# aconley/mbb_emcee

Measured on AMD Instinct MI355X. Metric: walker-likelihood evals/sec (+ MCMC steps/sec), 250 walkers × 8 bands, 1/2/4/8 GPU, higher is better.
Workload: dtype f64; 1 GPU; cfg2/cfg3: 8 passbands (NQ 2209) with full response integration, thick+alpha, 250 walkers per GPU, device-resident stretch move; 1 step = 2 dependent half-steps; walkers_per_gpu=250, walkers=250, bands=8, nq=2209, sampler_form=form 7: one launch per <=4096 steps, preconditioning=50 ms of scratch-ensemble steps before the W warm-up steps (GPU clocks)

## Files before the change

mbb_emcee_amd/csrc/mbb_flowm.hip.h:

```cpp
#pragma once
#include "mbb_kernels.hip.h"

__device__ __forceinline__ long long flow_spin_limit(int spec_cfg)
{
    const int v = (spec_cfg >> 24) & 0x3f;
    return v == 63 ? 0ll : 1ll << (v ? v : 22);
}

constexpr int kFmReady = 0;
constexpr int kFmQDone = 4;
constexpr int kFmEDone = 8;
constexpr int kFmPen = 16;
constexpr int kFmStaged = 12;

__device__ __forceinline__ int fm_loop_lane(int l)
{
    asm volatile("" : "+v"(l));
    return l;
}
__device__ __forceinline__ void fm_put(double *pair, double v, unsigned long long tag)
{
    typedef unsigned int u32x4 __attribute__((ext_vector_type(4)));
    const unsigned long long vb = (unsigned long long)__double_as_longlong(v), chk = tag ^ vb;
    const u32x4 d = {(unsigned int)vb, (unsigned int)(vb >> 32), (unsigned int)chk, (unsigned int)(chk >> 32)};
    asm volatile("global_store_dwordx4 %0, %1, off sc1" : : "v"(pair), "v"(d) : "memory");
}
__device__ __forceinline__ bool fm_get(const double *pair, unsigned long long tag, double &v)
{
    typedef unsigned int u32x4 __attribute__((ext_vector_type(4)));
    u32x4 d;
    asm volatile("global_load_dwordx4 %0, %1, off sc1\n\ts_waitcnt vmcnt(0)" : "=v"(d) : "v"(pair) : "memory");
    const unsigned long long vb = ((unsigned long long)d.y << 32) | d.x, chk = ((unsigned long long)d.w << 32) | d.z;
    v = __longlong_as_double((long long)vb);
    return (chk ^ vb) == tag;
}

#define MBB_FM_COMMON() \
    const int nun = a.nunit, npart = a.npart, nb = a.nb; \
    const int wbase = ((int)blockIdx.x >> 1) * NP, cand = (int)blockIdx.x & 1; \
    WalkerK *wk0 = reinterpret_cast<WalkerK *>(smem_raw); \
    double *partial0 = reinterpret_cast<double *>(wk0 + NP * kFmNB); \
    double *mflux_all = partial0 + NP * kFmNB * (size_t)npart; \
    double *prop0 = mflux_all + 2 * nb; \
    double *s_flux = prop0 + NP * kFmNB * kFmProp; \
    double *s_ivar = s_flux + nb; \
    double *s_invcov = s_ivar + nb; \
    int2 *s_band = reinterpret_cast<int2 *>(s_invcov + (a.cov_in_lds ? (size_t)nb * nb : 0)); \
    double *cscr = reinterpret_cast<double *>(s_band + nb + 1); \
    int *ctl0 = reinterpret_cast<int *>(cscr + kFmNC * 64); \
    const size_t tab_off = ((size_t)(reinterpret_cast<unsigned char *>(ctl0 + 32 * NP) - smem_raw) + 15) & ~(size_t)15; \
    double *s_nu = reinterpret_cast<double *>(smem_raw + tab_off); \
    double *s_lnnu = s_nu + (STAGE ? a.nchunk * 64 : 0); \
    double *s_wt = s_lnnu + (STAGE ? a.nchunk * 64 : 0); \
    const long long spin_limit = flow_spin_limit(a.spec_cfg); \
    const FlowMView fv = flowm_view(a.spec, a.nw); \
    const unsigned long long serial32 = a.flow_serial << 32; \
    unsigned long long *const done_set = fv.done + (size_t)(a.spec_cfg & 1) * kFmRing * 16; \
    const int niter = a.persist;
#define MBB_FM_PAIRS_LOOP _Pragma("clang loop unroll(disable)")
#define MBB_FM_PAIR(vp) \
    const int w = wbase + (vp); \
    if constexpr (NP > 1) { if (w >= a.n) continue; }       \
    WalkerK *const wk = wk0 + (vp) * kFmNB; \
    double *const partial = partial0 + (size_t)(vp) * kFmNB * npart; \
    double *const prop = prop0 + (vp) * kFmNB * kFmProp; \
    int *const ctl = ctl0 + 32 * (vp); \
    (void)wk; (void)partial; (void)prop; (void)ctl
#define MBB_FM_ORDER() do { __builtin_amdgcn_fence(__ATOMIC_ACQ_REL, "wavefront"); __builtin_amdgcn_wave_barrier(); } while (0)
#define MBB_FM_WAITS() \
    auto dec_ok = [&](unsigned long long v, unsigned long long need) {    \
        return (v >> 32) == (serial32 >> 32) && ((v & 0xffffffffull) >> 1) >= need; \
    }; \
    auto lds_wait = [&](int *word, int need) { \
        long long spins = 0; \
        while (__hip_atomic_load(word, __ATOMIC_RELAXED, __HIP_MEMORY_SCOPE_WORKGROUP) < need) { \
            ++spins; \
            if (spins > spin_limit * 16 || \
                ((spins & 255) == 8 && __hip_atomic_load(a.errflag, __ATOMIC_RELAXED, __HIP_MEMORY_SCOPE_AGENT) != 0)) { \
                atomicMax(a.errflag, 9); \
                break; \
            } \
            __builtin_amdgcn_s_sleep(1); \
        } \
        MBB_FM_ORDER(); \
    }; \
    auto lds_post = [&](int *word, int v) { \
        MBB_FM_ORDER(); \
        __hip_atomic_store(word, v, __ATOMIC_RELAXED, __HIP_MEMORY_SCOPE_WORKGROUP); \
    }; \
    (void)dec_ok; (void)lds_wait; (void)lds_post
#ifdef MBB_WAVE_VECTOR
#define MBB_WAVE_ID(t) ((t) >> 6)
#else
#define MBB_WAVE_ID(t) __builtin_amdgcn_readfirstlane((t) >> 6)
#endif

template <bool OPTHIN, bool NOALPHA, bool STAGE, int NP>
__global__ void __launch_bounds__(1024) k_flowm(const LikeArgs a)
{
    static_assert(NP == 1, "one pair of walkers per workgroup (the two-pair shape is not built or tested any more)");
    CLikeArgs *const ka = MBB_KERNARGS();
    extern __shared__ __align__(16) unsigned char smem_raw[];
    __shared__ __align__(16) double s_tab[kExp2N];
    __shared__ __align__(16) double s_pb[kPolyBDoubles];
    __shared__ __align__(16) double s_pc[OPTHIN ? 2 : kPolyCDoubles];
    const int tid = threadIdx.x, lane = tid & 63, wave = MBB_WAVE_ID(tid);
    const int nwave = blockDim.x >> 6, nq = nwave - kFmNC - 2;
    const bool spread = nwave == 16;
    const int role = spread ? ((wave & 3) == 3 ? 1 + (wave >> 2) : (wave == 14 ? 2 + kFmNC : 0))
                            : (wave < nq ? 0 : 1 + wave - nq);
    const int qi = spread ? wave - (wave >> 2) : wave;
    {
        MBB_ROLE_ARGS();
        MBB_FM_COMMON();
        if (tid < 32 * NP) ctl0[tid] = 0;
        if (cand == 0 && tid < 12 * NP && wbase + tid / 12 < a.n) {
            const int t12 = tid % 12;
            const int r = (t12 < 6 ? 0 : a.c_count) + wbase + tid / 12, e = t12 < 6 ? t12 : t12 - 6;
            fm_put(fv.row + (size_t)r * kFmWords + 2 * e, a.pos6[(size_t)r * 6 + e], serial32);
        }
        if (blockIdx.x == 0 && tid < kFmRing * 16)
            __hip_atomic_store(fv.done + (size_t)((a.spec_cfg & 1) ^ 1) * kFmRing * 16 + tid, 0ull, __ATOMIC_RELAXED, __HIP_MEMORY_SCOPE_AGENT);
        (void)done_set; (void)niter; (void)spin_limit;
    }
    __syncthreads();
#ifdef MBB_STAMPS
    if (tid == 0 && a.stamps) a.stamps[(1u << 20) + 4096 + blockIdx.x] = __builtin_amdgcn_s_memrealtime();
    unsigned long long t_acc[8] = {0, 0, 0, 0, 0, 0, 0, 0};
    unsigned long long t_last = __builtin_amdgcn_s_memtime();
#define FM_T(kk) do { const unsigned long long t_now = __builtin_amdgcn_s_memtime(); t_acc[kk] += t_now - t_last; t_last = t_now; } while (0)
#define FM_TD(kk, dep) do { asm volatile("" ::"v"(dep)); FM_T(kk); } while (0)
#define FM_TOUT() do { if (lane == 0 && a.stamps) for (int kk = 0; kk < 8; ++kk) a.stamps[((size_t)blockIdx.x * 16 + wave) * 8 + kk] = t_acc[kk]; } while (0)
    if (lane == 0 && a.stamps) {
        unsigned hwid, xcc;
        asm volatile("s_getreg_b32 %0, hwreg(HW_REG_HW_ID)" : "=s"(hwid));
        asm volatile("s_getreg_b32 %0, hwreg(HW_REG_XCC_ID)" : "=s"(xcc));
        a.stamps[(1u << 20) + blockIdx.x * 16 + wave] = ((unsigned long long)xcc << 32) | hwid;
    }
#define FM_EV(jj, ev) do { if (lane == 0 && a.stamps && (jj) >= niter - 64) \
        a.stamps[(1u << 20) + 8192 + (((size_t)blockIdx.x * 64 + ((jj) & 63)) * 16 + (ev))] = __builtin_amdgcn_s_memrealtime(); } while (0)
#define FM_EVV(jj, ev, val) do { if (lane == 0 && a.stamps && (jj) >= niter - 64) \
        a.stamps[(1u << 20) + 8192 + (((size_t)blockIdx.x * 64 + ((jj) & 63)) * 16 + (ev))] = (unsigned long long)(val); } while (0)
#else
#define FM_EV(jj, ev) do { } while (0)
#define FM_EVV(jj, ev, val) do { } while (0)
#define FM_T(kk) do { } while (0)
#define FM_TD(kk, dep) do { } while (0)
#define FM_TOUT() do { } while (0)
#endif

    if (role == 0 || role > kFmNC) {
        MBB_ROLE_ARGS();
        MBB_FM_COMMON();
        MBB_FM_WAITS();
        const int ns = nq + 2, si = role == 0 ? qi : nq + (role - 1 - kFmNC);
        const int t0 = si * 64 + lane, nt = ns * 64;
        const double2 *gb = reinterpret_cast<const double2 *>(a.poly_b);
        const double2 *gc = reinterpret_cast<const double2 *>(a.poly_c);
        double2 *lb = reinterpret_cast<double2 *>(s_pb);
        double2 *lc = reinterpret_cast<double2 *>(s_pc);
        for (int i = t0; i < kExp2N; i += nt) s_tab[i] = kExp2Tab[i];
        for (int i = t0; i < kPolyBDoubles / 2; i += nt) lb[i] = gb[i];
        if (!OPTHIN)
            for (int i = t0; i < kPolyCDoubles / 2; i += nt) lc[i] = gc[i];
        for (int bb = t0; bb < nb; bb += nt) { s_flux[bb] = a.flux[bb]; s_ivar[bb] = a.ivar[bb]; s_band[bb] = a.band_rng[bb]; }
        if (a.cov_in_lds)
            for (int i = t0; i < nb * nb; i += nt) s_invcov[i] = a.invcov[i];
        if (STAGE) {
            const int n2 = a.nchunk * 32;
            const double2 *g0 = reinterpret_cast<const double2 *>(a.nu), *g1 = reinterpret_cast<const double2 *>(a.lnnu),
                          *g2 = reinterpret_cast<const double2 *>(a.wt);
            double2 *l0 = reinterpret_cast<double2 *>(s_nu), *l1 = reinterpret_cast<double2 *>(s_lnnu),
                    *l2 = reinterpret_cast<double2 *>(s_wt);
            for (int i = t0; i < n2; i += nt) { l0[i] = g0[i]; l1[i] = g1[i]; l2[i] = g2[i]; }
        }
        asm volatile("s_waitcnt vmcnt(0) lgkmcnt(0)" ::: "memory");
        MBB_FM_ORDER();
        if (lane == 0) __hip_atomic_fetch_add(ctl0 + kFmStaged, 1, __ATOMIC_RELAXED, __HIP_MEMORY_SCOPE_WORKGROUP);
        lds_wait(ctl0 + kFmStaged, ns);
    }
    if (role != 0) __builtin_amdgcn_s_setprio(3);
    if (role == 0) {
        MBB_ROLE_ARGS();
        MBB_FM_COMMON();
        MBB_FM_WAITS();
        MBB_PIN(a.unit_tab); MBB_PIN(a.tail_slot); MBB_PIN(a.errflag);
        if (!STAGE) { MBB_PIN(a.nu); MBB_PIN(a.lnnu); MBB_PIN(a.wt); }
        auto T_nu = [&](int i) { if constexpr (STAGE) return s_nu[i]; else return a.nu[i]; };
        auto T_ln = [&](int i) { if constexpr (STAGE) return s_lnnu[i]; else return a.lnnu[i]; };
        auto T_wt = [&](int i) { if constexpr (STAGE) return s_wt[i]; else return a.wt[i]; };
        const SampleTabs tabs = {s_tab, s_pb, s_pc};
        int4 us_first = make_int4(0, 0, 0, 0);
        if (qi < nun) us_first = a.unit_tab[qi];
        int tail_first = -1;
        if (qi < nun && us_first.w == 2) tail_first = a.tail_slot[4 * us_first.x + (lane >> 4)];
        for (int it = 0; it < niter; ++it)
        MBB_FM_PAIRS_LOOP
        for (int vp = 0; vp < NP; ++vp) {
            MBB_FM_PAIR(vp);
            const int b = it & (kFmNB - 1);
            lds_wait(ctl + kFmReady + b, it + 1);
            FM_T(0);
            if (qi == 1) FM_EV(it, 14);
            const WalkerK *wkb = wk + b;
            double *part = partial + (size_t)b * npart;
            if (wkb->status == ROW_OK) {
                const WalkerK k = *wkb;
                for (int u = qi; u < nun; u += nq) {
                    const int4 us = (u == qi) ? us_first : a.unit_tab[u];
                    const int s = us.x, c0 = us.y, c1 = us.z;
                    double acc = 0.0;
                    int c = c0;
                    for (; c + 2 <= c1; c += 2) {
                        const int i0 = c * 64 + lane, i1 = i0 + 64;
                        const double n0 = T_nu(i0), l0 = T_ln(i0), q0 = T_wt(i0);
                        const double n1 = T_nu(i1), l1 = T_ln(i1), q1 = T_wt(i1);
                        const double f0 = fnu_sample<OPTHIN, NOALPHA, true, false>(k, n0, l0, &tabs);
                        const double f1 = fnu_sample<OPTHIN, NOALPHA, true, false>(k, n1, l1, &tabs);
                        acc = fma(f0, q0, acc);
                        acc = fma(f1, q1, acc);
                    }
                    if (c < c1) {
                        const int i = c * 64 + lane;
                        const double f = fnu_sample<OPTHIN, NOALPHA, true, false>(k, T_nu(i), T_ln(i), &tabs);
                        acc = fma(f, T_wt(i), acc);
                    }
                    if (us.w == 0) {
                        acc = wave_sum_l63(acc);
                        if (lane == 63) part[s] = acc;
                    } else if (us.w == 2) {
                        acc = row_sum(acc);
                        if ((lane & 15) == 0) {
                            const int sl = (u == qi) ? tail_first : a.tail_slot[4 * s + (lane >> 4)];
                            if (sl >= 0) part[sl] = acc;
                        }
                    } else {
                        part[s + lane] = acc;
                    }
                }
            }
            MBB_FM_ORDER();
#ifdef MBB_STAMPS
            if (lane == 0) {
                const int cnt = __hip_atomic_fetch_add(ctl + kFmQDone + b, 1, __ATOMIC_RELAXED, __HIP_MEMORY_SCOPE_WORKGROUP);
                if (cnt + 1 == nq * ((it / kFmNB) + 1)) FM_EV(it, 15);
            }
#else
            if (lane == 0) __hip_atomic_fetch_add(ctl + kFmQDone + b, 1, __ATOMIC_RELAXED, __HIP_MEMORY_SCOPE_WORKGROUP);
#endif
            FM_T(1);
        }
        FM_TOUT();
        return;
    }

    if (role > kFmNC) {
        MBB_ROLE_ARGS();
        MBB_FM_COMMON();
        MBB_FM_WAITS();
        MBB_PIN(a.n); MBB_PIN(a.nw); MBB_PIN(a.c_count); MBB_PIN(a.step); MBB_PIN(a.seed); MBB_PIN(a.stretch_a);
        MBB_PIN(a.has_gprior); MBB_PIN(a.invcov); MBB_PIN(a.cov_in_lds); MBB_PIN(a.pos6); MBB_PIN(a.chain6);
        MBB_PIN(a.nacc); MBB_PIN(a.errflag);
        double *mflux = mflux_all + (size_t)(role - 1 - kFmNC) * nb;
        for (int it = role - 1 - kFmNC; it < niter; it += 2)
        MBB_FM_PAIRS_LOOP
        for (int vp = 0; vp < NP; ++vp) {
            MBB_FM_PAIR(vp);
            const int b = it & (kFmNB - 1);
            const int L_step = a.step + (it >> 1), L_half = it & 1;
            const unsigned long long L_seed = a.seed + 0x9E3779B97F4A7C15ull * (unsigned long long)(it >> 1);
            const int row = (L_half ? a.c_count : 0) + w, c_begin = L_half ? 0 : a.c_count;
            double zz, u3;
            int pj;
            stretch_draw(row, L_step, L_half, L_seed, a.stretch_a, a.c_count, zz, pj, u3);
            const int prow = c_begin + pj;
            const int m_par = flow_cnt(L_half ^ 1, it), m_s = flow_cnt(L_half, it);
            const unsigned long long need_p = (unsigned long long)flow_seq(L_half ^ 1, m_par);
            const double *lnp_p = fv.row + ((size_t)(m_s % kFmSlots) * a.nw + row) * kFmWords + 10;
            const unsigned long long tag_s = serial32 | (unsigned long long)flow_seq(L_half, m_s);
            const unsigned long long need_g = 2ull * (unsigned long long)a.n * (unsigned long long)(((it - kFmLag) / kFmRing) + 1);
            const unsigned long long *word = lane == 22 ? fv.mseq + (size_t)prow * kFmMseq + (m_par % kFmSlots)
                                                        : done_set + ((it - kFmLag) & (kFmRing - 1)) * 16;
            const bool watch = (lane == 22 && need_p > 0) || (lane == 23 && it >= kFmLag);
            const WalkerK *wkb = wk + b;
            const double *pr = prop + b * kFmProp;
            int st = ROW_SKIP;
            double cbb = 0.0, pen_u = 0.0, pen_g = 0.0, lnz4 = 0.0, lnu = 0.0, acc = 0.0;
            double q[5] = {0.0, 0.0, 0.0, 0.0, 0.0}, old5[5] = {0.0, 0.0, 0.0, 0.0, 0.0};
            auto sums = [&]() {
                lds_wait(ctl + kFmPen + b, it + 1);
                st = wkb->status;
                cbb = wkb->cq; pen_u = pr[7]; pen_g = pr[8];
#pragma unroll
                for (int i = 0; i < 5; ++i) { q[i] = pr[i]; old5[i] = pr[9 + i]; }
                lnz4 = pr[5]; lnu = pr[6];
                if (st == ROW_OK) {
                    const double *pj2 = partial + (size_t)b * npart;
                    auto band = [&](const int bb) {
                        double sum = 0.0;
                        const int2 rng = s_band[bb];
                        for (int sg = rng.x; sg < rng.y; sg += 4) {
                            const int l = rng.y - 1;
                            const double q0 = pj2[sg], q1 = pj2[min(sg + 1, l)], q2 = pj2[min(sg + 2, l)], q3 = pj2[min(sg + 3, l)];
                            sum += q0;
                            if (sg + 1 < rng.y) sum += q1;
                            if (sg + 2 < rng.y) sum += q2;
                            if (sg + 3 < rng.y) sum += q3;
                        }
                        sum *= cbb;
                        const double d = s_flux[bb] - sum;
                        if (a.invcov) mflux[bb] = d;
                        else acc = fma(d * d, s_ivar[bb], acc);
                    };
                    for (int bb = lane; bb < nb; bb += 64) band(bb);
                    if (a.invcov) {
                        MBB_FM_ORDER();
                        for (int i = lane; i < nb; i += 64) {
                            double t = 0.0;
                            const double *crow = (a.cov_in_lds ? s_invcov : a.invcov) + (size_t)i * nb;
                            for (int jj = 0; jj < nb; ++jj) t = fma(crow[jj], mflux[jj], t);
                            acc = fma(mflux[i], t, acc);
                        }
                    }
                    acc = (nb <= 16) ? wave_sum_row0(acc) : wave_sum(acc);
                }
                MBB_FM_ORDER();
                if (lane == 0) lds_post(ctl + kFmEDone + b, it + 1);
            };
            const int q_need = nq * ((it / kFmNB) + 1);
            FM_EV(it, 9);
#ifdef MBB_STAMPS
            unsigned long long t_ok = 0;
#endif
            unsigned long long pv = 0;
            double lnp = 0.0;
            bool ok = !(watch || lane == 21), have_sums = false;
            long long spins = 0;
            for (;;) {
                double lv = 0.0;
                unsigned long long lchk = 0, wv = 0;
                const bool ask_l = lane == 21 && !ok, ask_w = watch && !ok;
                if (ask_l) {
                    lv = ld_dev(lnp_p);
                    lchk = __hip_atomic_load(reinterpret_cast<const unsigned long long *>(lnp_p) + 1, __ATOMIC_RELAXED, __HIP_MEMORY_SCOPE_AGENT);
                }
                if (ask_w) wv = __hip_atomic_load(word, __ATOMIC_RELAXED, __HIP_MEMORY_SCOPE_AGENT);
                if (!have_sums && __hip_atomic_load(ctl + kFmQDone + b, __ATOMIC_RELAXED, __HIP_MEMORY_SCOPE_WORKGROUP) >= q_need) {
                    MBB_FM_ORDER();
                    FM_EV(it, 4);
                    sums();
                    have_sums = true;
                }
                if (ask_l) { lnp = lv; ok = (lchk ^ (unsigned long long)__double_as_longlong(lv)) == tag_s; }
                if (ask_w) { pv = wv; ok = lane == 22 ? dec_ok(pv, need_p) : pv >= need_g; }
#ifdef MBB_STAMPS
                if ((ask_l || ask_w) && ok) t_ok = __builtin_amdgcn_s_memrealtime();
#endif
                if (__builtin_amdgcn_ballot_w64(!ok) == 0) break;
                ++spins;
                if (spins > spin_limit ||
                    ((spins & 255) == 8 && __hip_atomic_load(a.errflag, __ATOMIC_RELAXED, __HIP_MEMORY_SCOPE_AGENT) != 0)) {
                    atomicMax(a.errflag, 9);
                    break;
                }
                __builtin_amdgcn_s_sleep(1);
            }
            const int flag = (need_p > 0 && (__shfl(pv, 22) & 1ull)) ? 1 : 0;
            const bool mine = flag == cand;
            const double lnp_cur = __shfl(lnp, 21);
            FM_TD(0, lnp_cur);
            FM_EV(it, 5);
            FM_EVV(it, 7, prow);
#ifdef MBB_STAMPS
            { const unsigned long long t21 = __shfl(t_ok, 21), t22 = __shfl(t_ok, 22), t23 = __shfl(t_ok, 23);
              FM_EVV(it, 10, t21); FM_EVV(it, 11, t22); FM_EVV(it, 12, t23); }
#endif
            if (!have_sums) {
                lds_wait(ctl + kFmQDone + b, q_need);
                FM_T(1);
                FM_EV(it, 4);
                sums();
            }
            FM_TD(2, acc);
            {
                double r;
                if (st == ROW_BELOW_LOWLIM) r = -__builtin_inf();
                else if (st != ROW_OK) r = __builtin_nan("");
                else {
                    r = fma(-0.5, acc, pen_u);
                    if (a.has_gprior) r += pen_g;
                }
                if (mine) {
                    if (lane == 0 && (st >= 2 || r != r)) atomicMax(a.errflag, (st >= 2 && st <= (int)ROW_NONFINITE) ? st : (int)ROW_NONFINITE);
                    const bool accept = (lnz4 + r - lnp_cur) > lnu;
                    const int m_new = m_s + 1;
                    FM_EV(it, 6);
                    if (lane == 0)
                        __hip_atomic_store(fv.mseq + (size_t)row * kFmMseq + (m_new % kFmSlots),
                                           serial32 | (2ull * (unsigned long long)(it + 1) + (accept ? 1ull : 0ull)), __ATOMIC_RELAXED,
                                           __HIP_MEMORY_SCOPE_AGENT);
                    const double lnp_new = accept ? r : lnp_cur;
                    double ve = lnp_new;
#pragma unroll
                    for (int i = 0; i < 5; ++i) ve = ((lane & 7) == i) ? (accept ? q[i] : old5[i]) : ve;
                    if (lane < 6) {
                        fm_put(fv.row + ((size_t)(m_new % kFmSlots) * a.nw + row) * kFmWords + 2 * lane, ve,
                               serial32 | (unsigned long long)(it + 1));
                        if (it + 2 >= niter) a.pos6[(size_t)row * 6 + lane] = ve;
                    }
                    else if (lane >= 8 && lane < 14 && a.chain6)
                        a.chain6[((size_t)it * a.n + w) * 6 + (lane - 8)] = ve;
                    if (lane == 0 && accept) atomicAdd(a.nacc + (size_t)L_half * a.n + w, 1u);
                }
                if (lane == 0) __hip_atomic_fetch_add(done_set + (it & (kFmRing - 1)) * 16, 1ull, __ATOMIC_RELAXED, __HIP_MEMORY_SCOPE_AGENT);
            }
            FM_T(3);
        }
        FM_TOUT();
        return;
    }

    {
        MBB_ROLE_ARGS();
        MBB_FM_COMMON();
        MBB_FM_WAITS();
        MBB_PIN(a.c_count); MBB_PIN(a.step); MBB_PIN(a.seed); MBB_PIN(a.stretch_a); MBB_PIN(a.nw); MBB_PIN(a.errflag); MBB_PIN(a.zpow);
        MBB_PIN(a.lowlim[0]); MBB_PIN(a.lowlim[1]); MBB_PIN(a.lowlim[2]); MBB_PIN(a.lowlim[3]); MBB_PIN(a.lowlim[4]);
        MBB_PIN(a.nunorm); MBB_PIN(a.lnunorm); MBB_PIN(a.has_uplim); MBB_PIN(a.has_gprior);
        const int cb = role - 1;
        const int lane_w = lane;
        double *scr = cscr + (size_t)cb * 64;
        auto spin = [&](const unsigned long long *word, unsigned long long need, bool watch) {
            unsigned long long v = 0;
            long long spins = 0;
            for (;;) {
                bool ok = true;
                if (watch) { v = __hip_atomic_load(word, __ATOMIC_RELAXED, __HIP_MEMORY_SCOPE_AGENT); ok = dec_ok(v, need); }
                if (__builtin_amdgcn_ballot_w64(!ok) == 0) break;
                ++spins;
                if (spins > spin_limit ||
                    ((spins & 255) == 8 && __hip_atomic_load(a.errflag, __ATOMIC_RELAXED, __HIP_MEMORY_SCOPE_AGENT) != 0)) {
                    atomicMax(a.errflag, 9);
                    break;
                }
                __builtin_amdgcn_s_sleep(1);
            }
            return v;
        };
        for (int j = cb; j < niter; j += kFmNC)
        MBB_FM_PAIRS_LOOP
        for (int vp = 0; vp < NP; ++vp) {
            MBB_FM_PAIR(vp);
            const int lane = fm_loop_lane(lane_w);
            const int vrow = lane >> 4, l16 = lane & 15, base = lane & 48;
            const int hj = j & 1;
            const int sb = hj ? a.c_count : 0, ob = hj ? 0 : a.c_count;
            const int tn = a.step + (j >> 1);
            const unsigned long long seed_n = a.seed + 0x9E3779B97F4A7C15ull * (unsigned long long)(j >> 1);
            const int tp = a.step + ((j - 1) >> 1), hp = hj ^ 1;
            const unsigned long long seed_p = a.seed + 0x9E3779B97F4A7C15ull * (unsigned long long)((j - 1) >> 1);
            const bool c1 = cand && j > 0;
            const int rown = sb + w;
            double zz = 1.0, u3 = 0.5, zp = 1.0, up;
            int pj = 0, pjp = 0;
            stretch_draw(rown, tn, hj, seed_n, a.stretch_a, a.c_count, zz, pj, u3);
            if (c1) stretch_draw(ob + pj, tp, hp, seed_p, a.stretch_a, a.c_count, zp, pjp, up);
            const int m_s = flow_cnt(hj, j - 1), m_o = flow_cnt(hj ^ 1, j - 1);
            const int m_next = m_s + 1;
            const int g = j - 2;
            const int m_q = flow_cnt(hj ^ 1, g);
            const int pprow = sb + pjp, prow = ob + pj;
            int qr = 0, qp = 0;
            if (m_s > 0) {
                const int tg = a.step + (g >> 1);
                const unsigned long long seed_g = a.seed + 0x9E3779B97F4A7C15ull * (unsigned long long)(g >> 1);
                double u0, z0;
                stretch_draw(rown, tg, hj, seed_g, a.stretch_a, a.c_count, z0, qr, u0);
                if (c1) stretch_draw(pprow, tg, hj, seed_g, a.stretch_a, a.c_count, z0, qp, u0);
            }
            int snv_off = 0, cpv_off = 15;
            {
                const bool has = m_s > 0;
                const int so = (has ? m_s - 1 : 0) % kFmSlots;
                const unsigned long long tag_old = serial32 | (unsigned long long)flow_seq(hj, has ? m_s - 1 : 0);
                const unsigned long long tag_g = serial32 | (unsigned long long)(g + 1);
                const unsigned long long tag_o = serial32 | (unsigned long long)flow_seq(hj ^ 1, m_o);
                const double *src = fv.row;
                unsigned long long tag = 0, need = 0;
                const unsigned long long *wsrc = fv.mseq;
                int slot = -1, kind = 0;
                if (lane < 2) {
                    const int r = lane == 0 ? qr : qp;
                    wsrc = fv.mseq + (size_t)(ob + r) * kFmMseq + (m_q % kFmSlots);
                    need = (unsigned long long)flow_seq(hj ^ 1, m_q);
                    kind = (has && m_q > 0 && (lane == 0 || c1)) ? 1 : 0;
                } else if (lane < 7) {
                    src = fv.row + ((size_t)so * a.nw + rown) * kFmWords + 2 * (lane - 2); tag = tag_old; slot = lane - 2; kind = 2;
                } else if (lane < 12) {
                    src = fv.row + ((size_t)so * a.nw + pprow) * kFmWords + 2 * (lane - 7); tag = tag_old; slot = 15 + lane - 7; kind = c1 ? 2 : 0;
                } else if (lane < 17) {
                    src = fv.row + ((size_t)(m_o % kFmSlots) * a.nw + prow) * kFmWords + 2 * (lane - 12); tag = tag_o; slot = 30 + lane - 12; kind = 2;
                } else if (lane < 27) {
                    const int c = (lane - 17) / 5, i = (lane - 17) - 5 * c;
                    src = fv.prop + (((size_t)rown * kFmSlots + (m_s % kFmSlots)) * 2 + c) * kFmWords + 2 * i; tag = tag_g; slot = 5 + lane - 17;
                    kind = has ? 2 : 0;
                } else if (lane < 37) {
                    const int c = (lane - 27) / 5, i = (lane - 27) - 5 * c;
                    src = fv.prop + (((size_t)pprow * kFmSlots + (m_s % kFmSlots)) * 2 + c) * kFmWords + 2 * i; tag = tag_g; slot = 20 + lane - 27;
                    kind = (has && c1) ? 2 : 0;
                }
                FM_EV(j, 13);
                bool ok = kind == 0;
                double v = 0.0;
                unsigned long long dv = 0;
                long long spins = 0;
                for (;;) {
                    if (kind == 2 && !ok) ok = fm_get(src, tag, v);
                    if (kind == 1 && !ok) { dv = __hip_atomic_load(wsrc, __ATOMIC_RELAXED, __HIP_MEMORY_SCOPE_AGENT); ok = dec_ok(dv, need); }
                    if (__builtin_amdgcn_ballot_w64(!ok) == 0) break;
                    ++spins;
                    if (spins > spin_limit ||
                        ((spins & 255) == 8 && __hip_atomic_load(a.errflag, __ATOMIC_RELAXED, __HIP_MEMORY_SCOPE_AGENT) != 0)) {
                        atomicMax(a.errflag, 9);
                        break;
                    }
                    __builtin_amdgcn_s_sleep(1);
                }
                if (slot >= 0) scr[slot] = v;
                FM_TD(0, v);
                FM_EV(j, 0);
                FM_EVV(j, 8, (unsigned long long)prow | ((unsigned long long)pprow << 10) | ((unsigned long long)(ob + qr) << 20) |
                                 ((unsigned long long)(ob + qp) << 30) | ((unsigned long long)(c1 ? 1 : 0) << 40) | ((unsigned long long)(m_s > 0 ? 1 : 0) << 41));
                MBB_FM_ORDER();
                const int cr = (int)(__shfl(dv, 0) & 1ull), cp = (int)(__shfl(dv, 1) & 1ull);
                const bool ar_v = has && (vrow & 1), ap_v = has && c1 && (vrow & 2);
                snv_off = ar_v ? 5 + 5 * cr : 0;
                cpv_off = ap_v ? 20 + 5 * cp : 15;
            }
            double snv[5], cpos[5], cpv[5];
#pragma unroll
            for (int i = 0; i < 5; ++i) { snv[i] = scr[snv_off + i]; cpv[i] = scr[cpv_off + i]; cpos[i] = scr[30 + i]; }
            FM_T(1);
            if (c1) {
#pragma unroll
                for (int i = 0; i < 5; ++i) cpos[i] = stretch_q(cpv[i], cpos[i], zp);
            }
            double p[5];
#pragma unroll
            for (int i = 0; i < 5; ++i) p[i] = stretch_q(cpos[i], snv[i], zz);
            double lo[4];
            vlog<true>(lo, p[0], p[2], zz, u3);
            WalkerK k;
            k.hokt9 = k.lhokt9 = k.beta = k.bp3 = k.cq = k.alpha = k.lx0 = k.xmerge = k.cbb = k.cpl = k.kap = k.peak = 0.0;
            k.status = ROW_SKIP;
            k.pad = 0;
            double pen_u = 0.0, pen_g = 0.0;
            const double lT = lo[0], lL = lo[1];
            const unsigned long long *w2 = fv.mseq + (size_t)(l16 == 0 ? rown : pprow) * kFmMseq + (m_s % kFmSlots);
            const bool watch2 = m_s > 0 && (l16 == 0 || (l16 == 1 && c1));
            const unsigned long long need2 = (unsigned long long)flow_seq(hj, m_s);
            unsigned long long v2 = 0;
#define MBB_WC_AFTER_PROLOGUE if (watch2) v2 = __hip_atomic_load(w2, __ATOMIC_RELAXED, __HIP_MEMORY_SCOPE_AGENT);
#define MBB_WC_PENALTIES_LATER
#include "mbb_walker_consts.inc"
#undef MBB_WC_PENALTIES_LATER
#undef MBB_WC_AFTER_PROLOGUE
#ifdef MBB_STAMPS
            {
                asm volatile("" ::"v"(pen_u + pen_g + k.cbb));
                const unsigned long long dt = __builtin_amdgcn_s_memtime() - t_last;
                if (dt > t_acc[6]) t_acc[6] = dt;
                if (t_acc[7] == 0 || dt < t_acc[7]) t_acc[7] = dt;
            }
#endif
            FM_TD(2, pen_u + pen_g + k.cbb);
            FM_EV(j, 1);
            if (__builtin_amdgcn_ballot_w64(watch2 && !dec_ok(v2, need2)) != 0) v2 = spin(w2, need2, watch2);
            const bool ar = m_s > 0 && (__shfl(v2, base + 0) & 1ull), ap = m_s > 0 && c1 && (__shfl(v2, base + 1) & 1ull);
            const int vsel = (ar ? 1 : 0) | (ap ? 2 : 0);
            FM_TD(3, v2);
            FM_EV(j, 2);
            const int bj = j & (kFmNB - 1);
            if (j >= kFmNB) lds_wait(ctl + kFmEDone + bj, j - kFmNB + 1);
            FM_T(4);
            if (vrow == vsel && l16 == 0) {
                wk[bj] = k;
                double *pr = prop + bj * kFmProp;
#pragma unroll
                for (int i = 0; i < 5; ++i) { pr[i] = p[i]; pr[9 + i] = snv[i]; }
                pr[5] = a.zpow * lo[2];
                pr[6] = lo[3];
                lds_post(ctl + kFmReady + bj, j + 1);
#ifdef MBB_STAMPS
                if (a.stamps && j >= niter - 64)
                    a.stamps[(1u << 20) + 8192 + (((size_t)blockIdx.x * 64 + (j & 63)) * 16 + 3)] = __builtin_amdgcn_s_memrealtime();
#endif
                double *rec = fv.prop + (((size_t)rown * kFmSlots + (m_next % kFmSlots)) * 2 + cand) * kFmWords;
                const unsigned long long tag = serial32 | (unsigned long long)(j + 1);
#pragma unroll
                for (int i = 0; i < 5; ++i) fm_put(rec + 2 * i, p[i], tag);
            }
#include "mbb_walker_penalties.inc"
            if (vrow == vsel && l16 == 0) {
                double *pr = prop + bj * kFmProp;
                pr[7] = pen_u;
                pr[8] = pen_g;
                lds_post(ctl + kFmPen + bj, j + 1);
            }
            FM_T(5);
        }
        FM_TOUT();
    }
#undef FM_EV
#undef FM_EVV
#undef FM_T
#undef FM_TD
#undef FM_TOUT
}
```

mbb_emcee_amd/csrc/mbb_hip.hip:

```cpp
#include <hip/hip_runtime.h>
#include <dlfcn.h>
#include <math.h>
#include <stdint.h>
#include <stdio.h>
#include <stdlib.h>
#include <string.h>
#include <time.h>

#include <algorithm>
#include <functional>
#include <string>
#include <type_traits>
#include <atomic>
#include <chrono>
#include <mutex>
#include <thread>
#include <vector>

#include "../../include/mbb_hip.h"
#include "mbb_device.hip.h"
#include "mbb_kernels.hip.h"
#include "mbb_summary.hip.h"

#define MBB_FLOW_EXT(OT, NA)                                                    \
// ... 1188 lines not shown
        if ((rc = mbb_lnlike_batch(c, pos, R, lnp.data(), st.data(), nullptr))) return rc;
        for (int i = 0; i < R; ++i)
            if (st[i] >= 2) return fail(MBB_ERR_ARG, "initial position is not a valid SED or lnprob is NaN");
    }
    int nfree = 0;
    for (int src = 0; src < s->nsrc; ++src) {
        unsigned int mask = 0;
        const double *p0 = pos + (size_t)src * s->nw * 5;
        for (int w = 1; w < s->nw; ++w)
            for (int k = 0; k < 5; ++k)
                if (p0[(size_t)w * 5 + k] != p0[k]) mask |= 1u << k;
        const int nf = __builtin_popcount(mask);
        if (src > 0 && nf != nfree) return fail(MBB_ERR_ARG, "the sources' initial ensembles differ in the number of constant (fixed) columns");
        nfree = nf;
    }
    std::vector<double> rows((size_t)R * 6);
    for (int i = 0; i < R; ++i) {
        for (int k = 0; k < 5; ++k) rows[(size_t)i * 6 + k] = pos[(size_t)i * 5 + k];
        rows[(size_t)i * 6 + 5] = lnp[i];
        if (lnp[i] != lnp[i]) return fail(MBB_ERR_ARG, "initial lnprob is NaN");
    }
    HIPCHK(hipMemcpyAsync(s->d_pos6, rows.data(), rows.size() * sizeof(double),
                          hipMemcpyHostToDevice, c->stream));
    HIPCHK(hipStreamSynchronize(c->stream));
    if (s->lost || s->unchecked) {
        HIPCHK(hipMemset(s->d_err, 0, sizeof(int)));
        s->lost = s->unchecked = false;
        s->spec_form = 0;
    }
    s->zpow = nfree > 1 ? (double)(nfree - 1) : 0.0;
    return MBB_OK;
}

static int sampler_check_pending(mbb_ctx *c, mbb_sampler_state *s)
{
    if (s->unchecked) {
        int err = 0;
        HIPCHK(hipMemcpyAsync(&err, s->d_err, sizeof(int), hipMemcpyDeviceToHost, c->stream));
        HIPCHK(hipStreamSynchronize(c->stream));
        s->unchecked = false;
        if (err == 9) {
            HIPCHK(hipMemset(s->d_err, 0, sizeof(int)));
            s->lost = true;
            s->spec_form = 0;
        }
    }
    if (s->lost)
        return fail(MBB_ERR_STATE, "the one-launch sampler run timed out waiting for a half-step; the ensemble it "
                                   "left behind is not a state of the chain: set the sampler's state again");
    return MBB_OK;
}

struct ShardPlan { int shards, first, last, per; bool collective, xchg; };

static int shard_plan(const mbb_ctx *c, const mbb_sampler_state *s, ShardPlan &p)
{
    const int half = s->nw / 2;
    const bool xchg = c->x.connected && !s->pos6_owned && c->x.n > 1;
    p.collective = xchg || (c->comm != nullptr && c->nranks > 1);
    const int granks = xchg ? c->x.n : c->nranks, grank = xchg ? c->x.rank : c->rank;
    p.shards = p.collective ? granks : (int)(c->opt_vranks > 1 ? c->opt_vranks : 1);
    if (p.shards > 1 && s->nsrc > 1)
        return fail(MBB_ERR_ARG, "a sharded sampler run needs a single source");
    if (half % p.shards != 0)
        return fail(MBB_ERR_ARG, "nwalkers/2 must be a multiple of the number of ranks");
    p.per = half / p.shards;
    p.first = p.collective ? grank : 0;
    p.last = p.collective ? grank : p.shards - 1;
    p.xchg = xchg;
    return MBB_OK;
}

static int allgather_bytes(mbb_ctx *c, void *base, size_t bytes_per_rank)
{
    int r = g_rccl.AllGather((const char *)base + (size_t)c->rank * bytes_per_rank, base,
                             bytes_per_rank, 0 , c->comm, c->stream);
    if (r != 0) return fail(MBB_ERR_RCCL, g_rccl.GetErrorString ? g_rccl.GetErrorString(r) : "ncclAllGather failed");
    return MBB_OK;
}

struct RunPlan {
    ShardPlan p;
    int nl = 0;
    int form = 1;
    bool resting = false;
    int res_w = 1;
    int rows = 0, aw = 0, n_ahead = 0;
};

static int plan_sampler_run(const mbb_ctx *c, const mbb_sampler_state *s, int nsteps, bool one_launch_ok, RunPlan &rp)
{
    int rc = shard_plan(c, s, rp.p);
    if (rc) return rc;
    const ShardPlan &p = rp.p;
    const int nl = rp.nl = s->nsrc * p.per;
    int wpb, threads;
    pick_geometry(c, nl, wpb, threads);
    lookahead_plan(c, nl, threads, p.per, rp.rows, rp.aw, rp.n_ahead);
    const bool flow = one_launch_ok && c->opt_lookahead && c->opt_flow && s->nsrc == 1;
    if (flow && p.xchg && c->opt_xflow && nsteps > 0 && wpb == 1 && rp.n_ahead + nl <= c->cu_count &&
        (size_t)s->rows() <= c->x.cap_rows) {
        rp.form = 6;
        return MBB_OK;
    }
    const bool resident = flow && p.shards == 1 && !p.collective && nsteps >= (int)std::max<long>(1, c->opt_flow_min_steps);
    rp.res_w = c->opt_flowr_walkers > 0 ? (int)std::min<long>(c->opt_flowr_walkers, kFaMaxW) : (nl + c->cu_count - 1) / c->cu_count;
    const bool res_fits = rp.res_w >= 1 && rp.res_w <= kFaMaxW && (nl + rp.res_w - 1) / rp.res_w <= c->cu_count;
    if (resident && c->opt_flowm && c->opt_flowr != 2 && 2 * nl <= c->cu_count && wpb == 1) rp.form = 7;
    else if (resident && c->opt_flowr != 0 && res_fits) rp.form = 9;
    else rp.form = p.xchg ? 2 : 1;
    rp.resting = rp.form >= 7 && c->flow_rest > 0;
    if (rp.resting) rp.form = 1;
    return MBB_OK;
}

struct SamplerLaunch {
    double *pos6, *chain6;
    unsigned int *nacc;
    int *errflag;
    int s_begin, c_begin, c_count, m_count, nw, step, half, nw_src;
    double stretch_a, zpow;
    unsigned long long seed;
    int persist = 0, parity = 0;
    double *spec = nullptr;
    unsigned long long serial = 0;
};

static unsigned long long step_key(const mbb_sampler_state *s, int t)
{
    return s->seed + 0x9E3779B97F4A7C15ull * (s->steps_done + (unsigned long long)t + 1ull);
}

static int launch_sampler(mbb_ctx *c, const RunPlan &rp, const SamplerLaunch &sl, hipEvent_t *ev)
{
    if (c->nb <= 0) return fail(MBB_ERR_STATE, "bands not set (mbb_set_bands)");
    if (c->data_nb != c->nb) return fail(MBB_ERR_STATE, "data not set or band count mismatch");
    const int n = rp.nl, form = rp.form;
    LnlikeShape g;
    LikeArgs a;
    int rc = lnlike_shape(c, n, g, a);
    if (rc) return rc;
    a.pos6 = sl.pos6; a.chain6 = sl.chain6; a.nacc = sl.nacc; a.errflag = sl.errflag;
    a.s_begin = sl.s_begin; a.c_begin = sl.c_begin; a.c_count = sl.c_count; a.m_count = sl.m_count; a.nw = sl.nw;
    a.step = sl.step; a.half = sl.half; a.stretch_a = sl.stretch_a; a.zpow = sl.zpow; a.seed = sl.seed; a.nw_src = sl.nw_src;
    a.persist = sl.persist; a.spec = sl.spec; a.flow_serial = sl.serial;
    const int spin = (int)((c->opt_flow_spin_log2 & 0x3f) << 24);
    if (form == 7 || form == 9) {
        a.spec_cfg = spin | (sl.parity & 1);
        const bool fa = form == 9;
        const int W = fa ? rp.res_w : 1;
        const int wgs = fa ? (n + W - 1) / W : 2 * n;
        const int thr = fa ? 1024 : (std::min(g.threads / 64, 11) + 5) * 64;
        const size_t dyn_limit = dynamic_lds_limit(c), table_bytes = (size_t)c->nchunk * 64 * 3 * sizeof(double);
        auto lds_of = [&](bool cov) { return fa ? flowa_lds(c->nb, c->npart, cov, W) : flowm_lds(c->nb, c->npart, cov); };
        a.wpb = W;
        a.cov_in_lds = (c->has_cov && lds_of(true) <= std::min<size_t>(64 * 1024, dyn_limit)) ? 1 : 0;
        const size_t sm = lds_of(a.cov_in_lds != 0);
        const bool stg = c->opt_stage != 0 && sm + table_bytes + 16 <= dyn_limit;
        const size_t sm_total = sm + (stg ? table_bytes + 16 : 0);
        if (sm_total > dyn_limit) return fail(MBB_ERR_ARG, "band tables too large for the LDS plan");
        c->last_wpb = W; c->last_threads = thr; c->last_grid = wgs; c->last_smem = (long)sm_total;
        c->last_stage = stg ? 1 : 0; c->last_smode = form; c->last_ahead = 0;
        return launch_packed(c, kernel_slot(fa ? kFlowa : kFlowm, model_of(c), stg ? 1 : 0), wgs, thr, sm_total, a, ev);
    }
    int grid = g.grid;
    if (form == 2) a.xargs = c->x.d_args;
    if (form == 6) {
        a.spec_cfg = (rp.rows << 8) | (rp.aw << 16) | spin;
        a.n_ahead = rp.n_ahead;
        c->last_grid = grid += rp.n_ahead;
    }
    c->last_smode = form; c->last_ahead = form == 6 ? rp.n_ahead : 0;
    return launch_packed(c, kernel_slot(kLnlike, model_of(c), (form == 6 ? 3 : form) * 2 + (g.stage ? 1 : 0)), grid, g.threads,
                         g.smem, a, ev);
}

static int run_one_launch(mbb_ctx *c, mbb_sampler_state *s, const RunPlan &rp, SamplerLaunch &sl, int nsteps, bool store,
                          hipEvent_t *ev)
{
    const size_t R = (size_t)s->rows(), nl = (size_t)rp.nl;
    const bool sharded = rp.form == 6;
    const int rank = sharded ? c->x.rank : 0;
    double *const mine = sharded ? c->x.flow(rank) : nullptr;
    sl.spec = sharded ? reinterpret_cast<double *>(c->x.d_flowx) : s->d_spec;
    for (int t0 = 0; t0 < nsteps; t0 += 4096) {
        const int nt = std::min(4096, nsteps - t0);
        FlowX fxh;
        if (sharded) {
            memset(&fxh, 0, sizeof fxh);
            for (int r = 0; r < c->x.n; ++r) fxh.base[r] = c->x.flow(r);
            fxh.n = c->x.n; fxh.rank = rank; fxh.run = ++c->x.flow_run;
            HIPCHK(hipMemcpyAsync(c->x.d_flowx, &fxh, sizeof fxh, hipMemcpyHostToDevice, c->stream));
            hipLaunchKernelGGL(k_flow_init, dim3((unsigned)((R * 8 + 255) / 256)), dim3(256), 0, c->stream,
                               s->d_pos6, mine, (int)R);
            hipLaunchKernelGGL(k_flow_post, dim3(1), dim3(64), 0, c->stream, c->x.d_flowx, (int)R, 0, fxh.run,
                               (const int *)nullptr);
            HIPCHK(hipGetLastError());
        } else {
            sl.parity = s->flowm_parity;
            s->flowm_parity ^= 1;
        }
        sl.serial = ++g_flow_serial;
        sl.s_begin = rank * rp.p.per; sl.c_begin = s->nw / 2; sl.step = t0; sl.half = 0;
        sl.persist = 2 * nt;
        sl.chain6 = store ? s->d_chain6 + (((size_t)rank * nsteps + t0) * 2 * nl) * 6 : nullptr;
        sl.nacc = s->d_nacc + (size_t)rank * 2 * nl;
        sl.seed = step_key(s, t0);
        int rc = launch_sampler(c, rp, sl, ev);
        if (rc) return rc;
        if (sharded) {
            hipLaunchKernelGGL(k_flow_post, dim3(1), dim3(64), 0, c->stream, c->x.d_flowx, (int)R, 1, fxh.run,
                               (const int *)s->d_err);
            hipLaunchKernelGGL(k_flow_wait_end, dim3(1), dim3(64), 0, c->stream, flow_view(mine, (int)R).endf, c->x.n, rank,
                               fxh.run, c->x.spin_max, s->d_err);
            hipLaunchKernelGGL(k_flow_finish, dim3((unsigned)((R * 6 + 255) / 256)), dim3(256), 0, c->stream,
                               s->d_pos6, mine, (int)R, 2 * nt);
            HIPCHK(hipGetLastError());
        }
    }
    return MBB_OK;
}

static int run_train(mbb_ctx *c, mbb_sampler_state *s, const RunPlan &rp, SamplerLaunch &sl, int nsteps, bool store)
{
    const ShardPlan &p = rp.p;
    const size_t nl = (size_t)rp.nl;
    const int half = s->nw / 2;
    int rc;
    for (int t = 0; t < nsteps; ++t)
        for (int h = 0; h < 2; ++h) {
            const int hb = h ? half : 0;
            for (int r = p.first; r <= p.last; ++r) {
                sl.s_begin = hb + r * p.per; sl.c_begin = h ? 0 : half;
                sl.step = t; sl.half = h;
                sl.chain6 = store ? s->d_chain6 + ((((size_t)r * nsteps + t) * 2 + h) * nl) * 6 : nullptr;
                sl.nacc = s->d_nacc + ((size_t)r * 2 + h) * nl;
                sl.seed = step_key(s, t);
                if (p.xchg) ++c->x.seq;
                if ((rc = launch_sampler(c, rp, sl, nullptr))) return rc;
            }
            if (p.collective && !p.xchg &&
                (rc = allgather_bytes(c, s->d_pos6 + (size_t)hb * 6, (size_t)p.per * 6 * sizeof(double))))
                return rc;
        }
    if (p.xchg) {
        if (c->x.seq)
            hipLaunchKernelGGL(k_xchg_wait, dim3(1), dim3(64), 0, c->stream, c->x.flags(c->x.rank), c->x.n,
                               c->x.rank, c->x.seq, c->x.spin_max, s->d_err);
        HIPCHK(hipGetLastError());
    } else if (p.collective) {
        if (store && (rc = allgather_bytes(c, s->d_chain6, (size_t)nsteps * 2 * nl * 6 * sizeof(double)))) return rc;
        if ((rc = allgather_bytes(c, s->d_nacc, 2 * nl * sizeof(unsigned int)))) return rc;
    }
    return MBB_OK;
}

static int sampler_enqueue(mbb_ctx *c, mbb_sampler_state *s, const RunPlan &rp, int nsteps, double stretch_a, bool store,
                           bool backup, hipEvent_t *tev)
{
    s->backup_kept = false;
    if (rp.resting) --c->flow_rest;
    if (rp.form >= 7) {
        const size_t R = (size_t)s->rows();
        if (!s->d_spec) {
            HIPCHK(hipMalloc((void **)&s->d_spec, spec_words(R) * sizeof(double)));
            HIPCHK(hipMemsetAsync(s->d_spec, 0, spec_words(R) * sizeof(double), c->stream));
        }
        if (backup) {
            if (!s->d_bak) HIPCHK(hipMalloc((void **)&s->d_bak, R * 6 * sizeof(double) + R * sizeof(unsigned int)));
            HIPCHK(hipMemcpyAsync(s->d_bak, s->d_pos6, R * 6 * sizeof(double), hipMemcpyDeviceToDevice, c->stream));
            HIPCHK(hipMemcpyAsync(s->d_bak + R * 6, s->d_nacc, R * sizeof(unsigned int), hipMemcpyDeviceToDevice, c->stream));
        }
        s->backup_kept = backup;
        if (s->spec_form != 7 && s->spec_form != 9) {
            const FlowMView fvh = flowm_view(s->d_spec, (int)R);
            HIPCHK(hipMemsetAsync(fvh.done, 0, 2 * kFmRing * 16 * sizeof(unsigned long long), c->stream));
            s->flowm_parity = 0;
        }
        s->spec_form = rp.form;
    }
    const bool carried = tev && rp.form >= 7 && nsteps <= 4096;
    if (tev && !carried) HIPCHK(hipEventRecord(tev[0], c->stream));
    if (rp.p.xchg) {
        XchgArgs xa;
        memset(&xa, 0, sizeof xa);
        for (int r = 0; r < c->x.n; ++r) { xa.xpos[r] = c->x.pos6(r); xa.xflag[r] = c->x.flags(r); }
        xa.xcount = c->x.count(); xa.xn = c->x.n; xa.xrank = c->x.rank;
        xa.xseq0 = c->x.seq; xa.xspin_max = c->x.spin_max;
        HIPCHK(hipMemcpyAsync(c->x.d_args, &xa, sizeof xa, hipMemcpyHostToDevice, c->stream));
    }
    SamplerLaunch sl;
    sl.pos6 = s->d_pos6; sl.errflag = s->d_err; sl.nw = s->rows(); sl.nw_src = s->nw;
    sl.stretch_a = stretch_a; sl.zpow = s->zpow; sl.c_count = s->nw / 2; sl.m_count = rp.p.per;
    const int rc = rp.form >= 6 ? run_one_launch(c, s, rp, sl, nsteps, store, carried ? tev : nullptr)
                                : run_train(c, s, rp, sl, nsteps, store);
    if (rc) return rc;
    if (tev && !carried) HIPCHK(hipEventRecord(tev[1], c->stream));
    s->steps_done += (unsigned long long)nsteps;
    return MBB_OK;
}

static int summary_run(mbb_ctx *c, const double *d_chain, const double *d_lnprob, int nsrc, int nw, int nsteps,
                       const mbb_summary_spec *sp, const mbb_summary_out *o);

static int sampler_run(mbb_ctx *c, mbb_sampler_state *s, int nsteps, double stretch_a, double *chain, double *lnprob,
                       double *pos_out, double *lnprob_out, double *naccepted, bool one_launch_ok,
                       const mbb_summary_spec *sspec = nullptr, const mbb_summary_out *sout = nullptr)
// ... 957 lines not shown
```

mbb_emcee_amd/csrc/mbb_lds_plans.hip.h:

```cpp
#pragma once
#include <stddef.h>

#include "mbb_device.hip.h"
#include "mbb_flow_index.h"

constexpr int kFmProp = 16;
__host__ __device__ constexpr size_t flowm_lds(size_t nb, size_t npart, bool cov_in_lds, size_t np = 1)
{
    return np * kFmNB * sizeof(mbbd::WalkerK) +
           8 * (np * kFmNB * npart + 2 * nb + np * kFmNB * kFmProp + 2 * nb + (cov_in_lds ? nb * nb : 0)) +
           8 * (nb + 2) + 8 * (kFmNC * 64) + 128 * np + 32;
}

constexpr int kFaMaxW = 8;
constexpr int kFaNB = 2;
constexpr int kFaRec = 10;

__host__ __device__ constexpr size_t flowa_lds(size_t nb, size_t npart, bool cov_in_lds, size_t W)
{
    return kFaNB * W * (sizeof(mbbd::WalkerK) + 8 * npart + 8 * kFaRec) + 8 * W * nb + 8 * 2 * W * 8 + 16 * nb +
           (cov_in_lds ? 8 * nb * nb : 0) + 8 * (nb + 2) + 192 + 64;
}

constexpr unsigned long long kServeQuit = 0xffffull;

__host__ __device__ constexpr size_t serve_lds(size_t nb, size_t npart, bool cov_in_lds)
{
    return sizeof(mbbd::WalkerK) + 8 * npart + 8 * nb + 16 + 16 * nb + (cov_in_lds ? 8 * nb * nb : 0) + 8 * (nb + 2) + 64;
}
```

Before: 42.76 million evals/s.

## Stage unit tables in LDS, prefetch next unit, keep band data in registers

Copies the unit table and tail-slot table into LDS during staging, and prefetches the next unit's descriptor while the current unit is computed, so the integration loop no longer issues global loads. The reduction role keeps per-band ranges, flux and ivar in registers when nb<=64. The poll loop now reads the penalty record early and spins a bounded number of times before re-checking the global lnp and word values. Several cross-lane __shfl calls are replaced with readlane and DPP row broadcasts. This uses more LDS per workgroup, which grows with nunit, and changes the polling and sync timing.

```diff
diff --git a/mbb_emcee_amd/csrc/mbb_flowm.hip.h b/mbb_emcee_amd/csrc/mbb_flowm.hip.h
--- a/mbb_emcee_amd/csrc/mbb_flowm.hip.h
+++ b/mbb_emcee_amd/csrc/mbb_flowm.hip.h
@@ -12,6 +12,7 @@
 constexpr int kFmEDone = 8;
 constexpr int kFmPen = 16;
 constexpr int kFmStaged = 12;
+constexpr int kFmLooks = 8;
 
 __device__ __forceinline__ int fm_loop_lane(int l)
 {
@@ -33,6 +34,24 @@
     const unsigned long long vb = ((unsigned long long)d.y << 32) | d.x, chk = ((unsigned long long)d.w << 32) | d.z;
     v = __longlong_as_double((long long)vb);
     return (chk ^ vb) == tag;
+}
+
+template <int L>
+__device__ __forceinline__ unsigned int fm_lane_lo(unsigned long long v)
+{
+    return (unsigned int)__builtin_amdgcn_readlane((int)(unsigned int)v, L);
+}
+template <int L>
+__device__ __forceinline__ double fm_lane(double v)
+{
+    const int lo = __builtin_amdgcn_readlane(__double2loint(v), L), hi = __builtin_amdgcn_readlane(__double2hiint(v), L);
+    return __hiloint2double(hi, lo);
+}
+template <int N>
+__device__ __forceinline__ unsigned int fm_row_lo(unsigned long long v)
+{
+    const int lo = (int)(unsigned int)v;
+    return (unsigned int)__builtin_amdgcn_update_dpp(lo, lo, 0x150 + N, 0xf, 0xf, false);
 }
 
 #define MBB_FM_COMMON() \
@@ -48,7 +67,10 @@
     int2 *s_band = reinterpret_cast<int2 *>(s_invcov + (a.cov_in_lds ? (size_t)nb * nb : 0)); \
     double *cscr = reinterpret_cast<double *>(s_band + nb + 1); \
     int *ctl0 = reinterpret_cast<int *>(cscr + kFmNC * 64); \
-    const size_t tab_off = ((size_t)(reinterpret_cast<unsigned char *>(ctl0 + 32 * NP) - smem_raw) + 15) & ~(size_t)15; \
+    const size_t unit_off = ((size_t)(reinterpret_cast<unsigned char *>(ctl0 + 32 * NP) - smem_raw) + 15) & ~(size_t)15; \
+    int4 *s_unit = reinterpret_cast<int4 *>(smem_raw + unit_off);     \
+    int *s_tail = reinterpret_cast<int *>(s_unit + nun);               \
+    const size_t tab_off = unit_off + (size_t)kFmUnitBytes * nun; \
     double *s_nu = reinterpret_cast<double *>(smem_raw + tab_off); \
     double *s_lnnu = s_nu + (STAGE ? a.nchunk * 64 : 0); \
     double *s_wt = s_lnnu + (STAGE ? a.nchunk * 64 : 0); \
@@ -166,6 +188,11 @@
         for (int bb = t0; bb < nb; bb += nt) { s_flux[bb] = a.flux[bb]; s_ivar[bb] = a.ivar[bb]; s_band[bb] = a.band_rng[bb]; }
         if (a.cov_in_lds)
             for (int i = t0; i < nb * nb; i += nt) s_invcov[i] = a.invcov[i];
+        for (int u = t0; u < nun; u += nt) {
+            const int4 us = a.unit_tab[u];
+            s_unit[u] = us;
+            for (int r = 0; r < 4; ++r) s_tail[4 * u + r] = us.w == 2 ? a.tail_slot[4 * us.x + r] : -1;
+        }
         if (STAGE) {
             const int n2 = a.nchunk * 32;
             const double2 *g0 = reinterpret_cast<const double2 *>(a.nu), *g1 = reinterpret_cast<const double2 *>(a.lnnu),
@@ -204,10 +231,15 @@
             if (qi == 1) FM_EV(it, 14);
             const WalkerK *wkb = wk + b;
             double *part = partial + (size_t)b * npart;
-            if (wkb->status == ROW_OK) {
-                const WalkerK k = *wkb;
+            const WalkerK k = *wkb;
+            if (k.status == ROW_OK) {
+                int4 us = us_first;
+                int tail = tail_first;
                 for (int u = qi; u < nun; u += nq) {
-                    const int4 us = (u == qi) ? us_first : a.unit_tab[u];
+                    const bool more = u + nq < nun;
+                    int4 us_next = us;
+                    int tail_next = -1;
+                    if (more) { us_next = s_unit[u + nq]; tail_next = s_tail[4 * (u + nq) + (lane >> 4)]; }
                     const int s = us.x, c0 = us.y, c1 = us.z;
                     double acc = 0.0;
                     int c = c0;
@@ -230,12 +262,14 @@
                         if (lane == 63) part[s] = acc;
                     } else if (us.w == 2) {
                         acc = row_sum(acc);
-                        if ((lane & 15) == 0) {
-                            const int sl = (u == qi) ? tail_first : a.tail_slot[4 * s + (lane >> 4)];
-                            if (sl >= 0) part[sl] = acc;
-                        }
+                        if ((lane & 15) == 0 && tail >= 0) part[tail] = acc;
                     } else {
                         part[s + lane] = acc;
+                    }
+                    if (more) {
+                        us = make_int4(__builtin_amdgcn_readfirstlane(us_next.x), __builtin_amdgcn_readfirstlane(us_next.y),
+                                       __builtin_amdgcn_readfirstlane(us_next.z), __builtin_amdgcn_readfirstlane(us_next.w));
+                        tail = tail_next;
                     }
                 }
             }
@@ -262,6 +296,11 @@
         MBB_PIN(a.has_gprior); MBB_PIN(a.invcov); MBB_PIN(a.cov_in_lds); MBB_PIN(a.pos6); MBB_PIN(a.chain6);
         MBB_PIN(a.nacc); MBB_PIN(a.errflag);
         double *mflux = mflux_all + (size_t)(role - 1 - kFmNC) * nb;
+        const bool band_regs = nb <= 64;
+        int2 rng_r = make_int2(0, 0);
+        double flux_r = 0.0, ivar_r = 0.0;
+        if (band_regs && lane < nb) { rng_r = s_band[lane]; flux_r = s_flux[lane]; ivar_r = s_ivar[lane]; }
+        asm volatile("" : "+v"(rng_r.x), "+v"(rng_r.y), "+v"(flux_r), "+v"(ivar_r));
         for (int it = role - 1 - kFmNC; it < niter; it += 2)
         MBB_FM_PAIRS_LOOP
         for (int vp = 0; vp < NP; ++vp) {
@@ -287,18 +326,24 @@
             int st = ROW_SKIP;
             double cbb = 0.0, pen_u = 0.0, pen_g = 0.0, lnz4 = 0.0, lnu = 0.0, acc = 0.0;
             double q[5] = {0.0, 0.0, 0.0, 0.0, 0.0}, old5[5] = {0.0, 0.0, 0.0, 0.0, 0.0};
-            auto sums = [&]() {
-                lds_wait(ctl + kFmPen + b, it + 1);
+            bool have_rec = false;
+            auto record = [&]() {
                 st = wkb->status;
                 cbb = wkb->cq; pen_u = pr[7]; pen_g = pr[8];
 #pragma unroll
                 for (int i = 0; i < 5; ++i) { q[i] = pr[i]; old5[i] = pr[9 + i]; }
                 lnz4 = pr[5]; lnu = pr[6];
+                have_rec = true;
+            };
+            auto sums = [&]() {
+                if (!have_rec) {
+                    lds_wait(ctl + kFmPen + b, it + 1);
+                    record();
+                }
                 if (st == ROW_OK) {
                     const double *pj2 = partial + (size_t)b * npart;
-                    auto band = [&](const int bb) {
+                    auto band = [&](const int bb, const int2 rng, const double flux, const double ivar) {
                         double sum = 0.0;
-                        const int2 rng = s_band[bb];
                         for (int sg = rng.x; sg < rng.y; sg += 4) {
                             const int l = rng.y - 1;
                             const double q0 = pj2[sg], q1 = pj2[min(sg + 1, l)], q2 = pj2[min(sg + 2, l)], q3 = pj2[min(sg + 3, l)];
@@ -308,11 +353,15 @@
                             if (sg + 3 < rng.y) sum += q3;
                         }
                         sum *= cbb;
-                        const double d = s_flux[bb] - sum;
+                        const double d = flux - sum;
                         if (a.invcov) mflux[bb] = d;
-                        else acc = fma(d * d, s_ivar[bb], acc);
+                        else acc = fma(d * d, ivar, acc);
                     };
-                    for (int bb = lane; bb < nb; bb += 64) band(bb);
+                    if (band_regs) {
+                        if (lane < nb) band(lane, rng_r, flux_r, ivar_r);
+                    } else {
+                        for (int bb = lane; bb < nb; bb += 64) band(bb, s_band[bb], s_flux[bb], s_ivar[bb]);
+                    }
                     if (a.invcov) {
                         MBB_FM_ORDER();
                         for (int i = lane; i < nb; i += 64) {
@@ -337,20 +386,32 @@
             bool ok = !(watch || lane == 21), have_sums = false;
             long long spins = 0;
             for (;;) {
-                double lv = 0.0;
-                unsigned long long lchk = 0, wv = 0;
+                double lv;
+                unsigned long long lchk, wv;
                 const bool ask_l = lane == 21 && !ok, ask_w = watch && !ok;
                 if (ask_l) {
                     lv = ld_dev(lnp_p);
                     lchk = __hip_atomic_load(reinterpret_cast<const unsigned long long *>(lnp_p) + 1, __ATOMIC_RELAXED, __HIP_MEMORY_SCOPE_AGENT);
                 }
                 if (ask_w) wv = __hip_atomic_load(word, __ATOMIC_RELAXED, __HIP_MEMORY_SCOPE_AGENT);
-                if (!have_sums && __hip_atomic_load(ctl + kFmQDone + b, __ATOMIC_RELAXED, __HIP_MEMORY_SCOPE_WORKGROUP) >= q_need) {
-                    MBB_FM_ORDER();
-                    FM_EV(it, 4);
-                    sums();
-                    have_sums = true;
-                }
+#pragma nounroll
+                for (int look = 0; !have_sums; ++look) {
+                    if (!have_rec && __hip_atomic_load(ctl + kFmPen + b, __ATOMIC_RELAXED, __HIP_MEMORY_SCOPE_WORKGROUP) >= it + 1) {
+                        MBB_FM_ORDER();
+                        record();
+                    }
+                    if (__hip_atomic_load(ctl + kFmQDone + b, __ATOMIC_RELAXED, __HIP_MEMORY_SCOPE_WORKGROUP) >= q_need) {
+                        MBB_FM_ORDER();
+                        FM_EV(it, 4);
+                        sums();
+                        have_sums = true;
+                        break;
+                    }
+                    if (look >= kFmLooks) break;
+                    __builtin_amdgcn_s_sleep(1);
+                }
+                if (ask_l) asm volatile("" : "+v"(lv), "+v"(lchk));
+                if (ask_w) asm volatile("" : "+v"(wv));
                 if (ask_l) { lnp = lv; ok = (lchk ^ (unsigned long long)__double_as_longlong(lv)) == tag_s; }
                 if (ask_w) { pv = wv; ok = lane == 22 ? dec_ok(pv, need_p) : pv >= need_g; }
 #ifdef MBB_STAMPS
@@ -365,9 +426,9 @@
                 }
                 __builtin_amdgcn_s_sleep(1);
             }
-            const int flag = (need_p > 0 && (__shfl(pv, 22) & 1ull)) ? 1 : 0;
+            const int flag = (need_p > 0 && (fm_lane_lo<22>(pv) & 1u)) ? 1 : 0;
             const bool mine = flag == cand;
-            const double lnp_cur = __shfl(lnp, 21);
+            const double lnp_cur = fm_lane<21>(lnp);
             FM_TD(0, lnp_cur);
             FM_EV(it, 5);
             FM_EVV(it, 7, prow);
@@ -452,7 +513,7 @@
         for (int vp = 0; vp < NP; ++vp) {
             MBB_FM_PAIR(vp);
             const int lane = fm_loop_lane(lane_w);
-            const int vrow = lane >> 4, l16 = lane & 15, base = lane & 48;
+            const int vrow = lane >> 4, l16 = lane & 15;
             const int hj = j & 1;
             const int sb = hj ? a.c_count : 0, ob = hj ? 0 : a.c_count;
             const int tn = a.step + (j >> 1);
@@ -532,7 +593,7 @@
                 FM_EVV(j, 8, (unsigned long long)prow | ((unsigned long long)pprow << 10) | ((unsigned long long)(ob + qr) << 20) |
                                  ((unsigned long long)(ob + qp) << 30) | ((unsigned long long)(c1 ? 1 : 0) << 40) | ((unsigned long long)(m_s > 0 ? 1 : 0) << 41));
                 MBB_FM_ORDER();
-                const int cr = (int)(__shfl(dv, 0) & 1ull), cp = (int)(__shfl(dv, 1) & 1ull);
+                const int cr = (int)(fm_lane_lo<0>(dv) & 1u), cp = (int)(fm_lane_lo<1>(dv) & 1u);
                 const bool ar_v = has && (vrow & 1), ap_v = has && c1 && (vrow & 2);
                 snv_off = ar_v ? 5 + 5 * cr : 0;
                 cpv_off = ap_v ? 20 + 5 * cp : 15;
@@ -576,7 +637,7 @@
             FM_TD(2, pen_u + pen_g + k.cbb);
             FM_EV(j, 1);
             if (__builtin_amdgcn_ballot_w64(watch2 && !dec_ok(v2, need2)) != 0) v2 = spin(w2, need2, watch2);
-            const bool ar = m_s > 0 && (__shfl(v2, base + 0) & 1ull), ap = m_s > 0 && c1 && (__shfl(v2, base + 1) & 1ull);
+            const bool ar = m_s > 0 && (fm_row_lo<0>(v2) & 1u), ap = m_s > 0 && c1 && (fm_row_lo<1>(v2) & 1u);
             const int vsel = (ar ? 1 : 0) | (ap ? 2 : 0);
             FM_TD(3, v2);
             FM_EV(j, 2);
diff --git a/mbb_emcee_amd/csrc/mbb_hip.hip b/mbb_emcee_amd/csrc/mbb_hip.hip
--- a/mbb_emcee_amd/csrc/mbb_hip.hip
+++ b/mbb_emcee_amd/csrc/mbb_hip.hip
@@ -1364,7 +1364,7 @@
         const int wgs = fa ? (n + W - 1) / W : 2 * n;
         const int thr = fa ? 1024 : (std::min(g.threads / 64, 11) + 5) * 64;
         const size_t dyn_limit = dynamic_lds_limit(c), table_bytes = (size_t)c->nchunk * 64 * 3 * sizeof(double);
-        auto lds_of = [&](bool cov) { return fa ? flowa_lds(c->nb, c->npart, cov, W) : flowm_lds(c->nb, c->npart, cov); };
+        auto lds_of = [&](bool cov) { return fa ? flowa_lds(c->nb, c->npart, cov, W) : flowm_lds(c->nb, c->npart, cov, c->nunit); };
         a.wpb = W;
         a.cov_in_lds = (c->has_cov && lds_of(true) <= std::min<size_t>(64 * 1024, dyn_limit)) ? 1 : 0;
         const size_t sm = lds_of(a.cov_in_lds != 0);
diff --git a/mbb_emcee_amd/csrc/mbb_lds_plans.hip.h b/mbb_emcee_amd/csrc/mbb_lds_plans.hip.h
--- a/mbb_emcee_amd/csrc/mbb_lds_plans.hip.h
+++ b/mbb_emcee_amd/csrc/mbb_lds_plans.hip.h
@@ -5,11 +5,12 @@
 #include "mbb_flow_index.h"
 
 constexpr int kFmProp = 16;
-__host__ __device__ constexpr size_t flowm_lds(size_t nb, size_t npart, bool cov_in_lds, size_t np = 1)
+constexpr int kFmUnitBytes = 32;
+__host__ __device__ constexpr size_t flowm_lds(size_t nb, size_t npart, bool cov_in_lds, size_t nunit, size_t np = 1)
 {
     return np * kFmNB * sizeof(mbbd::WalkerK) +
            8 * (np * kFmNB * npart + 2 * nb + np * kFmNB * kFmProp + 2 * nb + (cov_in_lds ? nb * nb : 0)) +
-           8 * (nb + 2) + 8 * (kFmNC * 64) + 128 * np + 32;
+           8 * (nb + 2) + 8 * (kFmNC * 64) + 128 * np + 32 + kFmUnitBytes * nunit;
 }
 
 constexpr int kFaMaxW = 8;
```

After: 43.79 million evals/s, median of 6. 1.02x the previous value.
